# JuliaStats/Klara.jl

Hardware: AMD Instinct MI355X
Metric: MCMC transitions/sec (whole node), 100-dim Gaussian, 65k chains (higher is better)
Workload: dtype f64

## Files before the change

klara.jl_amd/csrc/klara_diagt.h:

```cpp
#pragma once
#include "klara_kernels.h"
#include "klara_mala_screen.h"

#ifndef KLARA_DIAGT_Q
#define KLARA_DIAGT_Q 8
#endif
#define KLARA_DIAGT_CPW (64 / KLARA_DIAGT_Q)
#ifndef KLARA_DT_FENCE_EVERY
#define KLARA_DT_FENCE_EVERY 2
#endif
#ifndef KLARA_DT_SLICE_WF
#define KLARA_DT_SLICE_WF 4
#endif
#ifndef KLARA_DT_W1
#define KLARA_DT_W1 4
#endif
#ifndef KLARA_Q4_MALA_WF
#define KLARA_Q4_MALA_WF 3
#endif
#ifndef KLARA_Q4_SCTAB_WF
#define KLARA_Q4_SCTAB_WF 3
#endif
#ifndef KLARA_DT_WF
#define KLARA_DT_WF 2
// ... 198 lines not shown
    constexpr int CH = KLARA_DT_RMW_CHUNK;
#pragma unroll
    for (int p0 = 0; p0 < NP; p0 += CH) {
        kd_uint4 ts[CH], tq[CH];
#pragma unroll
        for (int k = 0; k < CH; ++k) {
            if (p0 + k < NP) {
                const unsigned o = fold ? pair_off<NP, Q>(c, p0 + k) : KLARA_BUF_OOB;
                ts[k] = __builtin_amdgcn_raw_buffer_load_b128(wsum, o, 0, 0);
                tq[k] = __builtin_amdgcn_raw_buffer_load_b128(wsq, o, 0, 0);
            }
        }
#pragma unroll
        for (int k = 0; k < CH; ++k) {
            if (p0 + k < NP) {
                const int p = p0 + k;
                const unsigned o = fold ? pair_off<NP, Q>(c, p) : KLARA_BUF_OOB;
                const double s0 = __builtin_bit_cast(double, kd_uint2{ ts[k].x, ts[k].y }) + hf * x[2 * p];
                const double s1 = __builtin_bit_cast(double, kd_uint2{ ts[k].z, ts[k].w }) + hf * x[2 * p + 1];
                const double q0 = __builtin_bit_cast(double, kd_uint2{ tq[k].x, tq[k].y }) + hf * (x[2 * p] * x[2 * p]);
                const double q1 = __builtin_bit_cast(double, kd_uint2{ tq[k].z, tq[k].w }) + hf * (x[2 * p + 1] * x[2 * p + 1]);
                const kd_uint2 a = __builtin_bit_cast(kd_uint2, s0), b = __builtin_bit_cast(kd_uint2, s1);
                const kd_uint2 e = __builtin_bit_cast(kd_uint2, q0), f = __builtin_bit_cast(kd_uint2, q1);
                if (p < NP - 1) {
                    __builtin_amdgcn_raw_buffer_store_b128(kd_uint4{ a.x, a.y, b.x, b.y }, wsum, o, 0, 0);
                    __builtin_amdgcn_raw_buffer_store_b128(kd_uint4{ e.x, e.y, f.x, f.y }, wsq, o, 0, 0);
                } else {
                    const unsigned o1 = (fold && c.last_full) ? o + 8u : KLARA_BUF_OOB;
                    __builtin_amdgcn_raw_buffer_store_b64(a, wsum, o, 0, 0); __builtin_amdgcn_raw_buffer_store_b64(b, wsum, o1, 0, 0);
                    __builtin_amdgcn_raw_buffer_store_b64(e, wsq, o, 0, 0); __builtin_amdgcn_raw_buffer_store_b64(f, wsq, o1, 0, 0);
                }
            }
        }
    }
    held = fold ? 0 : held;
}

template <int NP, int Q>
__device__ __forceinline__ void load_pair_param(const PairCtx<NP, Q>& c, const gdouble* base, int D, double dflt, double (&v)[2 * NP])
{
#pragma unroll
    for (int p = 0; p < NP; ++p) {
        const int i = 2 * (p * Q + c.q);
        v[2 * p] = dflt; v[2 * p + 1] = dflt;
        if (base != nullptr && i < D) v[2 * p] = base[i];
        if (base != nullptr && i + 1 < D) v[2 * p + 1] = base[i + 1];
    }
}

template <int Q> struct PairShare {
    static constexpr int STEP = Q <= 8 ? 8 / Q : 0;
    static constexpr bool second(int p) { return STEP != 0 && ((p / (STEP ? STEP : 1)) & 1) != 0; }
};
template <int NP, int Q>
__device__ __forceinline__ void pair_words(const PairCtx<NP, Q>& c, unsigned long long seed, unsigned long long gchain,
                                           unsigned long long t, int p, uint32_t (&stash)[4], uint32_t& wa, uint32_t& wb)
{
    constexpr int STEP = PairShare<Q>::STEP, S1 = STEP ? STEP : 1;
    if (PairShare<Q>::second(p)) {
        wa = stash[2 * (p % S1)]; wb = stash[2 * (p % S1) + 1];
    } else {
        const uint32_t idx = (uint32_t)(p * Q + c.q);
        const bool pad = p == NP - 1 && !c.last_ok;
        const kd_u32x4 b = kd_stream_block(seed, gchain, t, pad ? idx : kd_pair_block(idx));
        if constexpr (STEP != 0) {
            wa = b.x; wb = b.y;
            stash[2 * (p % S1)] = b.z; stash[2 * (p % S1) + 1] = b.w;
        } else {
            const bool hb = !pad && kd_pair_half(idx) != 0u;
            wa = hb ? b.z : b.x; wb = hb ? b.w : b.y;
        }
    }
}
template <int NP, int Q, bool SCTAB = false>
__device__ __forceinline__ void pair_normals(const PairCtx<NP, Q>& c, unsigned long long seed, unsigned long long gchain,
                                             unsigned long long t, int p, uint32_t (&stash)[4], double& z0, double& z1, double& u1, double& lg1)
{
    uint32_t wa, wb;
    pair_words<NP, Q>(c, seed, gchain, t, p, stash, wa, wb);
    kd_normal_pair_w_t<SCTAB>(wa, wb, &z0, &z1, &u1, &lg1);
    KLARA_PIN(z0); KLARA_PIN(z1);
    if (p == NP - 1 && !c.last_ok) z0 = 0.0;
    if (p == NP - 1 && !c.last_full) z1 = 0.0;
}
template <int NP, int Q>
__device__ __forceinline__ void pair_issue(const PairCtx<NP, Q>& c, unsigned long long seed, unsigned long long gchain,
                                           unsigned long long t, int p, uint32_t (&stash)[4], kd_pair_reads& rd)
{
    uint32_t wa, wb;
    pair_words<NP, Q>(c, seed, gchain, t, p, stash, wa, wb);
    kd_normal_pair_issue(wa, wb, &rd);
    __builtin_amdgcn_sched_barrier(0);
}
template <int NP, int Q>
__device__ __forceinline__ void pair_issue_log(const PairCtx<NP, Q>& c, unsigned long long seed, unsigned long long gchain,
                                               unsigned long long t, int p, uint32_t (&stash)[4], kd_pair_reads& rd, uint32_t& wb)
{
    uint32_t wa;
    pair_words<NP, Q>(c, seed, gchain, t, p, stash, wa, wb);
    kd_normal_pair_issue_log(wa, wb, &rd);
    __builtin_amdgcn_sched_barrier(0);
}
__device__ __forceinline__ void pair_issue_angle(uint32_t wb, kd_pair_reads& rd)
{
    kd_normal_pair_issue_angle(wb, &rd);
    __builtin_amdgcn_sched_barrier(0);
}
template <int NP, int Q>
__device__ __forceinline__ void pair_finish(const PairCtx<NP, Q>& c, int p, const kd_pair_reads& rd, double& z0, double& z1, double& u1, double& lg1)
{
    kd_normal_pair_finish(&rd, &z0, &z1, &u1, &lg1);
    KLARA_PIN(z0); KLARA_PIN(z1);
    if (p == NP - 1 && !c.last_ok) z0 = 0.0;
    if (p == NP - 1 && !c.last_full) z1 = 0.0;
}

template <int V> struct kd_int { static constexpr int value = V; };
template <int FROM, int TO, class F>
__device__ __forceinline__ void kd_static_for(F&& f)
{
    if constexpr (FROM < TO) { f(kd_int<FROM>{}); kd_static_for<FROM + 1, TO>(f); }
}

template <bool UNITW>
__device__ __forceinline__ void diag_elem(double x, double w, double m2w, double m, double& term, double& grad)
{
    const double dd = UNITW ? x : x - m;
    term = UNITW ? dd * dd : w * (dd * dd);
    grad = UNITW ? -2.0 * dd : m2w * dd;
}

template <int SAMPLER, int NP, int Q, bool ONESTEP, bool TUNE, bool SCTAB = false>
__host__ __device__ constexpr int diagt_min_waves()
{
    return SCTAB && Q == 4 && NP > 8 ? KLARA_Q4_SCTAB_WF
         : NP <= 8 ? (ONESTEP && SAMPLER != KLARA_SAMPLER_HMC ? KLARA_DT_W1 : KLARA_DT_WF)
                   : (Q == 4 && NP <= 13 && !TUNE ? (SAMPLER == KLARA_SAMPLER_MALA ? KLARA_Q4_MALA_WF : 2) : 1);
}

#ifndef KLARA_SCTAB_MIN_STEPS
#define KLARA_SCTAB_MIN_STEPS 8
#endif
template <int SAMPLER, int NP, int Q, bool ONESTEP, bool UNITW, bool MON, bool TUNE>
__host__ __device__ constexpr bool diagt_sctab()
{
    return SAMPLER == KLARA_SAMPLER_MALA && ((Q == 4 && NP == 13) || (Q == 8 && NP == 7)) && !ONESTEP && UNITW && MON && !TUNE;
}
#ifndef KLARA_MALA_SCREEN
#define KLARA_MALA_SCREEN 1
#endif
#ifndef KLARA_MALA_SCREEN_RUN
#define KLARA_MALA_SCREEN_RUN 2
#endif
template <bool C, class A, class B> struct kd_type_if { typedef A type; };
template <class A, class B> struct kd_type_if<false, A, B> { typedef B type; };
template <int SAMPLER, int NP, int Q, bool UNITW, bool TUNE, bool USERPAIR, bool SCTAB>
__host__ __device__ constexpr bool diagt_mala_screen()
{
    return KLARA_MALA_SCREEN != 0 && SCTAB && SAMPLER == KLARA_SAMPLER_MALA && Q == 4 && NP == 13 && UNITW && !TUNE && !USERPAIR;
}
#ifndef KLARA_Q4_SCTAB_WG
#define KLARA_Q4_SCTAB_WG 256
#endif
template <int Q, bool SCTAB>
__host__ __device__ constexpr int diagt_wg_threads() { return SCTAB && Q == 4 ? KLARA_Q4_SCTAB_WG : 256; }
#ifndef KLARA_Q4_KEPT_MEANS
#define KLARA_Q4_KEPT_MEANS 0
#endif
#ifndef KLARA_Q8_KEPT_MEANS
#define KLARA_Q8_KEPT_MEANS 0
#endif
template <int SAMPLER, int NP, int Q, bool UNITW, bool TUNE, bool SCTAB>
__host__ __device__ constexpr int diagt_kept_means()
{
    return SCTAB && SAMPLER == KLARA_SAMPLER_MALA && UNITW && !TUNE ? (Q == 4 ? KLARA_Q4_KEPT_MEANS : Q == 8 ? KLARA_Q8_KEPT_MEANS : 0) : 0;
}

#ifdef KLARA_USER_PAIR_TARGET
#define KLARA_PAIR_CALL(a, b, P, g0, g1) klara_user_pair((a), (b), (P), D, (const double*)p.cdata, (long long)p.cndata, (g0), (g1))
#else
#define KLARA_PAIR_CALL(a, b, P, g0, g1) 0.0
#endif
template <int SAMPLER, int NP, int Q, bool ONESTEP, bool UNITW, bool MON, bool TUNE = false, bool DA = false, bool USERPAIR = false, bool SCTAB = false>
__global__ __launch_bounds__((diagt_wg_threads<Q, SCTAB>()), (SAMPLER == KLARA_SAMPLER_SLICE && NP <= 8 && !MON && !TUNE ? KLARA_DT_SLICE_WF : diagt_min_waves<SAMPLER, NP, Q, ONESTEP, TUNE, SCTAB>()))
void k_diagt(const KParams* __restrict__ pp, const KLaunch kl, const KAuto ka)
{
#ifndef KLARA_USER_PAIR_TARGET
    static_assert(!USERPAIR, "pair closures exist in run-time compiled translation units only");
#endif
    static_assert(!USERPAIR || (UNITW && Q >= 8), "pair closures: 8 or more lanes per chain");
    static_assert(!SCTAB || (!ONESTEP && !USERPAIR && SAMPLER != KLARA_SAMPLER_SLICE), "the remainder table: fused launches of the built-in MH / MALA / HMC kernels");
    if (ka.cell_in != nullptr && *ka.cell_in != ka.my_mode) return;
    static_assert(!(ONESTEP && (MON || TUNE)), "monitored / tuned jobs run the committing kernel");
    static_assert(!DA || (TUNE && SAMPLER == KLARA_SAMPLER_HMC), "dual averaging: tuned HMC");
    constexpr bool PLAIN = !TUNE;
    constexpr int E = 2 * NP, CPW = 64 / Q;
    constexpr bool NEEDG = SAMPLER == KLARA_SAMPLER_MALA || SAMPLER == KLARA_SAMPLER_HMC;
    constexpr bool SLICE = SAMPLER == KLARA_SAMPLER_SLICE;
    constexpr int KM = diagt_kept_means<SAMPLER, NP, Q, UNITW, TUNE, SCTAB>();
    static_assert(KM >= 0 && KM <= E, "kept drift means: a prefix of the lane's elements");
    constexpr bool SCREEN = diagt_mala_screen<SAMPLER, NP, Q, UNITW, TUNE, USERPAIR, SCTAB>();
    static_assert(!(SLICE && ONESTEP), "the slice sampler moves every chain: it runs the committing kernel");
    constexpr bool MEMSUM = MON && !TUNE && Q == 4 && (SAMPLER == KLARA_SAMPLER_MH || SAMPLER == KLARA_SAMPLER_MALA);
    const KParams& p = *pp;
    __shared__ __attribute__((aligned(16))) double lds_w[UNITW ? 2 : 2 * NP * Q];
    __shared__ __attribute__((aligned(16))) double lds_mu[UNITW ? 2 : 2 * NP * Q];
    __shared__ __attribute__((aligned(16))) double lds_m2w[UNITW ? 2 : 2 * NP * Q];
    if (!UNITW) {
        for (int i = (int)threadIdx.x; i < 2 * NP * Q; i += (int)blockDim.x) {
            lds_w[i] = (p.gw != nullptr && i < p.D) ? p.gw[i] : 1.0;
            lds_mu[i] = (p.gmu != nullptr && i < p.D) ? p.gmu[i] : 0.0;
            lds_m2w[i] = -2.0 * lds_w[i];
        }
    }
    __shared__ __attribute__((aligned(16))) double lds_screen[6];
    if constexpr (SCREEN) {
        if (threadIdx.x == 0) {
            const kd_mala_screen_k k = kd_mala_screen_consts(p.step0, p.sqrt_step0, 0.5 * p.inv_step0);
            lds_screen[0] = k.K0; lds_screen[1] = k.K1; lds_screen[4] = k.K2; lds_screen[5] = 0.0;
            lds_screen[2] = k.on ? k.T0 : __builtin_nan(""); lds_screen[3] = k.on ? k.T2 : __builtin_nan("");
        }
    }
    auto_begin();
    if constexpr (SCTAB) kd_sincos_rem_to_lds();
    kd_tables_to_lds();
    if (p.clock_probe != nullptr && blockIdx.x == (gridDim.x >> 1) && threadIdx.x == 0) {
        p.clock_probe[2] = __builtin_amdgcn_s_memtime(); p.clock_probe[3] = __builtin_amdgcn_s_memrealtime();
    }
    const int D = p.D;
    const PairCtx<NP, Q> cx = make_pctx<NP, Q>(D);
    const int nsteps = ONESTEP ? 1 : kl.nsteps;
    guchar* const accept_out = p.accept != nullptr ? p.accept + kl.t0 * (unsigned long long)p.nchains : nullptr;

    double sig[E];
    const auto wv = [&](int e) { return UNITW ? 1.0 : lds_w[2 * ((e >> 1) * Q + cx.q) + (e & 1)]; };
    const auto mv = [&](int e) { return UNITW ? 0.0 : lds_mu[2 * ((e >> 1) * Q + cx.q) + (e & 1)]; };
    const auto m2wv = [&](int e) { return UNITW ? -2.0 : lds_m2w[2 * ((e >> 1) * Q + cx.q) + (e & 1)]; };
    const auto wvl = [&](int e) { return UNITW ? 1.0 : *(volatile const double*)&lds_w[2 * ((e >> 1) * Q + cx.q) + (e & 1)]; };
    const auto mvl = [&](int e) { return UNITW ? 0.0 : *(volatile const double*)&lds_mu[2 * ((e >> 1) * Q + cx.q) + (e & 1)]; };
    const auto m2wvl = [&](int e) { return UNITW ? -2.0 : *(volatile const double*)&lds_m2w[2 * ((e >> 1) * Q + cx.q) + (e & 1)]; };
    if (SAMPLER == KLARA_SAMPLER_MH) load_pair_param<NP, Q>(cx, p.vecparam, D, 1.0, sig);
    const double gconst = USERPAIR ? 0.0 : p.gconst;

    const int acc_slot = (D + 1) >> 1;
    const bool acc_free = acc_slot < NP * Q && !PairShare<Q>::second(NP - 1);
    const int acc_lane = (cx.lane - cx.q) + (acc_slot & (Q - 1));

    const long long nwaves = (long long)gridDim.x * (blockDim.x >> 6);
    const long long wave0 = __builtin_amdgcn_readfirstlane((int)(blockIdx.x * (blockDim.x >> 6) + (threadIdx.x >> 6)));
    unsigned wave_acc = 0;
    KLARA_DT_GROUP_LOOP {
        const long long first_chain = grp * CPW;
        const long long left = p.nchains - first_chain;
        const int here = left < CPW ? (int)left : CPW;
        const bool chain_ok = cx.cw < here;
        const long long chain = first_chain + cx.cw;
        const unsigned long long gchain = (unsigned long long)(p.chain_offset + chain);
        const __amdgpu_buffer_rsrc_t wx = group_window(p.X, first_chain, here, D);
        const __amdgpu_buffer_rsrc_t wg = group_window(p.GR, first_chain, here, D);

        double x[E];
        load_pairs<NP, Q>(cx, wx, x);
        const auto late_ctx = [&]() -> PairCtx<NP, Q> {
            if constexpr (SCTAB && Q == 4) {
                int l = (int)__builtin_amdgcn_mbcnt_hi(~0u, __builtin_amdgcn_mbcnt_lo(~0u, 0u));
                KLARA_PIN(l);
                return make_pctx_at<NP, Q>(D, l & 63);
            } else return cx;
        };
        const auto user_pair = [&](int pi, double a, double b, double& nt, double& g0, double& g1) {
            double u0 = 0.0, u1 = 0.0, u = 0.0;
            const bool ok0 = pi < NP - 1 || cx.last_ok, ok1 = pi < NP - 1 || cx.last_full;
            if (ok0) u = KLARA_PAIR_CALL(a, b, pi * Q + cx.q, &u0, &u1);
            nt = ok0 ? -u : 0.0; g0 = ok0 ? u0 : 0.0; g1 = ok1 ? u1 : 0.0;
        };
        const auto grad_of = [&](const double (&v)[E], double (&out)[E]) {
            if constexpr (USERPAIR) {
#pragma unroll
                for (int pi = 0; pi < NP; ++pi) { double nt; user_pair(pi, v[2 * pi], v[2 * pi + 1], nt, out[2 * pi], out[2 * pi + 1]); }
            } else {
#pragma unroll
                for (int e = 0; e < E; ++e) { double term_; diag_elem<UNITW>(v[e], wv(e), m2wv(e), mv(e), term_, out[e]); }
            }
        };
        double lt = p.LT[chain_ok ? chain : 0];
        typename kd_type_if<SCREEN, unsigned, unsigned long long>::type nacc = 0;
        bool stuck = false;
        const bool do_sum = MON && p.sum != nullptr;
        double sm[MEMSUM ? 2 : E], sq[MEMSUM ? 2 : E];
        bool sums_loaded = false;
        long long held = 0;
        __amdgpu_buffer_rsrc_t wsum = wx, wsq = wx;
        if (do_sum) {
#pragma unroll
            for (int e = 0; e < (MEMSUM ? 2 : E); ++e) { sm[e] = 0.0; sq[e] = 0.0; }
            wsum = group_window(p.sum, first_chain, here, D); wsq = group_window(p.sumsq, first_chain, here, D);
            held = p.held[chain_ok ? chain : 0];
        }
        int sphase = kl.save_phase0;
        long long scol = kl.save_col0;
        const bool per_chain_tune = KCNT && !KPOOLED;
        const long long c0 = chain_ok ? chain : 0;
        TuneRegs tn;
        if (per_chain_tune) tn = { p.tune_step[c0], p.tune_accepted[c0], p.tune_proposed[c0], p.tune_totproposed[c0], 0, 0.0, 0.0 };
        else if (KPOOLED) tn = { p.tune_step[0], p.tune_accepted[0], 0, 0, 0, 0.0, 0.0 };
        else tn = { DA ? p.tune_step[c0] : p.step0, 0, 0, 0, 0, 0.0, 0.0 };
        if (DA) { tn.epsbar = p.da_epsbar[c0]; tn.hbar = p.da_hbar[c0]; }
        const long long acc0 = tn.accepted;
        tn.phase = per_chain_tune ? (int)(tn.proposed % p.period) : 0;

        struct { unsigned long long seed; long long hist_cols, held_inc; int thinning, acc_free, save_lo, save_hi; double sqrt_step0, half_inv_step0; } lc = {};
        if constexpr (SCTAB) {
            lc.seed = p.seed; lc.hist_cols = p.hist_cols; lc.thinning = (int)p.thinning;
            lc.held_inc = __builtin_amdgcn_readfirstlane(do_sum ? 1 : 0); lc.sqrt_step0 = p.sqrt_step0;
            KLARA_PIN_S(lc.seed); KLARA_PIN_S(lc.hist_cols); KLARA_PIN_S(lc.thinning);
            KLARA_PIN_S(lc.held_inc); KLARA_PIN_S(lc.sqrt_step0);
            const kd_uint2 hih = __builtin_bit_cast(kd_uint2, 0.5 * p.inv_step0);
            lc.half_inv_step0 = __builtin_bit_cast(double, kd_uint2{ (uint32_t)__builtin_amdgcn_readfirstlane((int)hih.x), (uint32_t)__builtin_amdgcn_readfirstlane((int)hih.y) });
            KLARA_PIN_S(lc.half_inv_step0);
            lc.acc_free = __builtin_amdgcn_readfirstlane(acc_free ? 1 : 0);
            KLARA_PIN_S(lc.acc_free);
            const long long lo = (long long)p.burnin - (long long)kl.t0, hi = (long long)p.nsteps_total - (long long)kl.t0;
            lc.save_lo = (int)(lo < 0 ? 0 : lo > nsteps ? nsteps : lo); lc.save_hi = (int)(hi < 0 ? 0 : hi > nsteps ? nsteps : hi);
            KLARA_PIN_S(lc.save_lo); KLARA_PIN_S(lc.save_hi);
        }
#define KLARA_LC(f) (SCTAB ? lc.f : p.f)
        double dm[KM > 0 ? KM : 1];
        const double neg_h_kept = KM > 0 ? -tn.step : 0.0;
        if constexpr (KM > 0) {
#pragma unroll
            for (int e = 0; e < KM; ++e) dm[e] = x[e] + neg_h_kept * x[e];
        }
        double sxx = 0.0;
        int srun = 0;
        if constexpr (SCREEN) {
#pragma unroll
            for (int e = 0; e < E; ++e) sxx = kd_fma(x[e], x[e], sxx);
        }
        for (int s = 0; s < nsteps; ++s) {
            const unsigned long long t = kl.t0 + (unsigned long long)s;
            if (KCNT) tune_count_proposal(p, tn);
            double xp[E];
            const auto put_xp = [&](int pi, double a, double b) { xp[2 * pi] = a; xp[2 * pi + 1] = b; };
            constexpr int NR = Q == 4 ? 2 : 1;
            double red[3 * NR] = {}, red1[1], red2[2];
            double u_last = 0.5, lg_last = 0.0;
            uint32_t nstash[4] = { 0u, 0u, 0u, 0u };
            bool acc;
            double ltp, a_da = 0.0;

            constexpr bool ZFIRST = (ONESTEP || Q != 4) && SAMPLER != KLARA_SAMPLER_HMC && !SLICE;
            double z[ZFIRST ? E : 2];
            kd_pair_reads rd[2];
            if (ZFIRST) {
                if constexpr (SCTAB) pair_issue<NP, Q>(cx, KLARA_LC(seed), gchain, t, 0, nstash, rd[0]);
#pragma unroll
                for (int pi = 0; pi < NP; ++pi) {
                    if constexpr (SCTAB) {
                        if (pi + 1 < NP) pair_issue<NP, Q>(cx, KLARA_LC(seed), gchain, t, pi + 1, nstash, rd[(pi + 1) & 1]);
                        pair_finish<NP, Q>(cx, pi, rd[pi & 1], z[2 * pi], z[2 * pi + 1], u_last, lg_last);
                        __builtin_amdgcn_sched_barrier(0);
                    } else {
                        pair_normals<NP, Q, SCTAB>(cx, KLARA_LC(seed), gchain, t, pi, nstash, z[2 * pi], z[2 * pi + 1], u_last, lg_last);
                        KLARA_DT_PAIR_FENCE(pi);
                    }
                }
            }
            if constexpr (SLICE) {
                if (do_sum && __any(held > 0))
                    diagt_fold<NP, Q>(cx, wsum, wsq, held > 0, sums_loaded, held, x, sm, sq);
            }
            if (SLICE) {
                acc = true;
                const __amdgpu_buffer_rsrc_t wwid = __builtin_amdgcn_make_buffer_rsrc((void*)p.vecparam, 0, D * 8, 0x00020000);
#pragma unroll
                for (int e = 0; e < E; ++e) {
                    const int i = 2 * ((e >> 1) * Q + cx.q) + (e & 1);
                    const bool live = chain_ok && i < D;
                    const uint32_t base = (uint32_t)(live ? i : 0) << KLARA_SLICE_ATT_BITS;
                    const kd_u32x4 b0 = kd_stream_block(KLARA_LC(seed), gchain, t, base);
                    const double lgu = kd_log_u01(kd_uniform_xy(b0));
                    const double ru = kd_uniform_zw(b0);
                    const double wi_t = UNITW ? 1.0 : wv(e), mi_t = UNITW ? 0.0 : mv(e);
                    const double xi = x[e], wd = __builtin_bit_cast(double, __builtin_amdgcn_raw_buffer_load_b64(wwid, (unsigned)(live ? i : 0) * 8u, 0, 0));
                    double tcur, gd_;
                    if constexpr (USERPAIR) { double g1_; user_pair(e >> 1, x[e & ~1], x[e | 1], tcur, gd_, g1_); }
                    else diag_elem<UNITW>(xi, wi_t, -2.0 * wi_t, mi_t, tcur, gd_);
                    double Li = xi - ru * wd;
                    double Ri = xi + (1.0 - ru) * wd;
                    const auto term_of = [&](double cand) -> double {
                        double tc, gd;
                        if constexpr (USERPAIR) { double g1; user_pair(e >> 1, (e & 1) ? x[e & ~1] : cand, (e & 1) ? cand : x[e | 1], tc, gd, g1); }
                        else diag_elem<UNITW>(cand, wi_t, -2.0 * wi_t, mi_t, tc, gd);
                        return tc;
                    };
                    if (p.stepout) {
                        double dl = tcur - term_of(Li);
                        int guard = 0;
                        while (true) {
                            bool go = live && !stuck && (dl > lgu);
                            if (go && ++guard > KLARA_SLICE_MAX_ATT) { stuck = true; go = false; }
                            if (!__any(go)) break;
                            const double Ln = Li - wd;
                            const double dn = tcur - term_of(go ? Ln : Li);
                            if (go) { Li = Ln; dl = dn; }
                        }
                        double dr = tcur - term_of(Ri);
                        guard = 0;
                        while (true) {
                            bool go = live && !stuck && (dr > lgu);
                            if (go && ++guard > KLARA_SLICE_MAX_ATT) { stuck = true; go = false; }
                            if (!__any(go)) break;
                            const double Rn = Ri + wd;
                            const double dn = tcur - term_of(go ? Rn : Ri);
                            if (go) { Ri = Rn; dr = dn; }
                        }
                    }
                    double xprime = xi;
                    bool done = !live || stuck;
                    kd_u32x4 ab = b0;
                    for (uint32_t a = 1;; ++a) {
                        if (!done && a > KLARA_SLICE_MAX_ATT) { stuck = true; done = true; }
                        if (!__any(!done)) break;
                        if (a & 1u) ab = kd_stream_block(KLARA_LC(seed), gchain, t, kd_slice_attempt_slot(base, a));
                        const double u = (a & 1u) ? kd_uniform_xy(ab) : kd_uniform_zw(ab);
                        const double cand = u * (Ri - Li) + Li;
                        const double tc = term_of(done ? xprime : cand);
                        if (!done) {
                            xprime = cand;
                            if (tcur - tc > lgu) done = true;
                            else if (cand > xi) Ri = cand;
                            else if (cand < xi) Li = cand;
                            else { stuck = true; done = true; }
                        }
                    }
                    if (live && !stuck) x[e] = xprime;
                }
                red1[0] = 0.0;
                if constexpr (USERPAIR) {
#pragma unroll
                    for (int pi = 0; pi < NP; ++pi) { double nt, g0_, g1_; user_pair(pi, x[2 * pi], x[2 * pi + 1], nt, g0_, g1_); red1[0] = red1[0] + nt; }
                } else {
#pragma unroll
                for (int e = 0; e < E; ++e) { double te, gd; diag_elem<UNITW>(x[e], wv(e), m2wv(e), mv(e), te, gd); red1[0] = red1[0] + te; }
                }
                group_allreduce<1>(red1, Q, cx.lane);
                lt = gconst - red1[0];
                ltp = lt;
#pragma unroll
                for (int e = 0; e < E; ++e) xp[e] = x[e];
            } else if (SAMPLER == KLARA_SAMPLER_MH) {
                const auto mh_elem = [&](int e, double ze, int r) -> double {
                    const double xe = x[e] + sig[e] * ze;
                    double term, gd;
                    diag_elem<UNITW>(xe, wv(e), m2wv(e), mv(e), term, gd);
                    red[r] = red[r] + term;
                    return xe;
                };
#pragma unroll
                for (int pi = 0; pi < NP; ++pi) {
                    double z0 = ZFIRST ? z[(2 * pi) % (ZFIRST ? E : 2)] : 0.0, z1 = ZFIRST ? z[(2 * pi + 1) % (ZFIRST ? E : 2)] : 0.0;
                    if (!ZFIRST) pair_normals<NP, Q, SCTAB>(cx, KLARA_LC(seed), gchain, t, pi, nstash, z0, z1, u_last, lg_last);
                    const int r = (NR == 2 && (pi & 1)) ? 3 : 0;
                    if constexpr (USERPAIR) {
                        const double a = x[2 * pi] + sig[2 * pi] * z0, b = x[2 * pi + 1] + sig[2 * pi + 1] * z1;
                        double nt, g0, g1;
                        user_pair(pi, a, b, nt, g0, g1);
                        red[r] = red[r] + nt;
                        put_xp(pi, a, b);
                    } else {
                        const double a = mh_elem(2 * pi, z0, r), b = mh_elem(2 * pi + 1, z1, r);
                        put_xp(pi, a, b);
                    }
                    if (!ZFIRST) KLARA_DT_PAIR_FENCE(pi);
                }
                if (NR == 2) {
                    red2[0] = red[0]; red2[1] = red[3];
                    group_allreduce<2>(red2, Q, cx.lane);
                    red1[0] = red2[0] + red2[1];
                } else {
                    red1[0] = red[0];
                    group_allreduce<1>(red1, Q, cx.lane);
                }
                ltp = gconst - red1[0];
                const double ratio = ltp - lt;
                acc = ratio > 0.0;
                if (acc_free) acc = acc || ratio > lane_bcast(lg_last, acc_lane);
                else if (!acc && ratio > KD_LOG_UMIN_GUARD)
                    acc = ratio > kd_log_u01(kd_accept_uniform(kd_stream_block(KLARA_LC(seed), gchain, t, (uint32_t)acc_slot)));
            } else if (SAMPLER == KLARA_SAMPLER_MALA) {
                const double h_ = tn.step, halfh = 0.5 * h_, sq = KCNT ? __builtin_sqrt(h_) : KLARA_LC(sqrt_step0);
                const double half_inv_h = SCTAB ? lc.half_inv_step0 : 0.5 * (KCNT ? 1.0 / h_ : p.inv_step0);
                const double neg_h = -h_;
                constexpr bool FROM_TERM = UNITW && PLAIN;
                const auto mala_elem = [&](int e, double ze, int r, bool first) -> double {
                    double term, ge = 0.0, gpe;
                    if constexpr (!UNITW) diag_elem<UNITW>(x[e], wv(e), m2wv(e), mv(e), term, ge);
                    const double m_ = UNITW ? (e < KM ? dm[e < KM ? e : 0] : x[e] + neg_h * x[e]) : x[e] + halfh * ge;
                    const double xe = m_ + sq * ze;
                    diag_elem<UNITW>(xe, wv(e), m2wv(e), mv(e), term, gpe);
                    red[r] = first ? term : red[r] + term;
                    const double q1 = m_ - xe;
                    red[r + 1] = first ? (q1 * q1) * half_inv_h : red[r + 1] + (q1 * q1) * half_inv_h;
                    const double mup = UNITW ? xe + neg_h * xe : xe + halfh * gpe;
                    const double q2 = mup - x[e];
                    red[r + 2] = first ? (q2 * q2) * half_inv_h : red[r + 2] + (q2 * q2) * half_inv_h;
                    return xe;
                };
                bool screened = false;
                if constexpr (SCREEN) {
                    double sxz = 0.0, szz = 0.0;
                    kd_screm_t sk01, skt;
                    double sk2;
                    pair_issue<NP, Q>(cx, KLARA_LC(seed), gchain, t, 0, nstash, rd[0]);
#pragma unroll
                    for (int pi = 0; pi < NP; ++pi) {
                        double z0, z1;
                        uint32_t wb_next = 0u;
                        if (pi == NP - 1) {
                            typedef volatile const __attribute__((address_space(3))) kd_screm_t* lds_entry;
                            sk01 = *(lds_entry)&lds_screen[0]; skt = *(lds_entry)&lds_screen[2];
                            sk2 = *(volatile const __attribute__((address_space(3))) double*)&lds_screen[4];
                            __builtin_amdgcn_sched_barrier(0);
                        }
                        if (pi + 1 < NP) pair_issue_log<NP, Q>(cx, KLARA_LC(seed), gchain, t, pi + 1, nstash, rd[(pi + 1) & 1], wb_next);
                        pair_finish<NP, Q>(cx, pi, rd[pi & 1], z0, z1, u_last, lg_last);
                        if (pi + 1 < NP) pair_issue_angle(wb_next, rd[(pi + 1) & 1]);
                        sxz = kd_fma(x[2 * pi], z0, sxz); sxz = kd_fma(x[2 * pi + 1], z1, sxz);
                        szz = kd_fma(z0, z0, szz); szz = kd_fma(z1, z1, szz);
                        put_xp(pi, z0, z1);
                        __builtin_amdgcn_sched_barrier(0);
                    }
                    double sc[2] = { kd_mala_screen_e(sk01.x, sk01.y, sk2, sxx, sxz, szz), kd_mala_screen_t(skt.x, skt.y, sxx, szz) };
                    group_allreduce<2>(sc, Q, cx.lane);
                    double lg_s;
                    if (lc.acc_free != 0) lg_s = lane_bcast(lg_last, acc_lane);
                    else { lg_s = KD_LOG_UMIN_GUARD; KLARA_PIN_S(lg_s); }
                    const bool certain = !chain_ok || kd_mala_screen_decide(sc[0], sc[1], lt, gconst, lg_s, nullptr, nullptr) != 0;
                    screened = __all(certain) != 0;
                    if (KLARA_MALA_SCREEN_RUN > 0 && srun >= KLARA_MALA_SCREEN_RUN) screened = false;
                    srun = screened ? srun + 1 : 0;
                    KLARA_PIN(srun);
                    acc = false; ltp = lt;
                }
                if (!screened) {
#pragma unroll
                for (int pi = 0; pi < NP; ++pi) {
                    double z0 = ZFIRST ? z[(2 * pi) % (ZFIRST ? E : 2)] : 0.0, z1 = ZFIRST ? z[(2 * pi + 1) % (ZFIRST ? E : 2)] : 0.0;
                    if constexpr (SCREEN) { z0 = xp[2 * pi]; z1 = xp[2 * pi + 1]; }
                    else if constexpr (!ZFIRST && SCTAB) {
                        if (pi == 0) pair_issue<NP, Q>(cx, KLARA_LC(seed), gchain, t, 0, nstash, rd[0]);
                        pair_finish<NP, Q>(cx, pi, rd[pi & 1], z0, z1, u_last, lg_last);
                        if (pi + 1 < NP) pair_issue<NP, Q>(cx, KLARA_LC(seed), gchain, t, pi + 1, nstash, rd[(pi + 1) & 1]);
                    } else if (!ZFIRST) pair_normals<NP, Q, SCTAB>(cx, KLARA_LC(seed), gchain, t, pi, nstash, z0, z1, u_last, lg_last);
                    const int r = (NR == 2 && (pi & 1)) ? 3 : 0;
                    if constexpr (USERPAIR) {
                        double nt, ge0, ge1, gp0, gp1;
                        user_pair(pi, x[2 * pi], x[2 * pi + 1], nt, ge0, ge1);
                        const double m0 = x[2 * pi] + halfh * ge0, m1 = x[2 * pi + 1] + halfh * ge1;
                        const double a = m0 + sq * z0, b = m1 + sq * z1;
                        user_pair(pi, a, b, nt, gp0, gp1);
                        red[r] = red[r] + nt;
                        const double q10 = m0 - a, q11 = m1 - b;
                        red[r + 1] = red[r + 1] + (q10 * q10) * half_inv_h;
                        red[r + 1] = red[r + 1] + (q11 * q11) * half_inv_h;
                        const double q20 = (a + halfh * gp0) - x[2 * pi], q21 = (b + halfh * gp1) - x[2 * pi + 1];
                        red[r + 2] = red[r + 2] + (q20 * q20) * half_inv_h;
                        red[r + 2] = red[r + 2] + (q21 * q21) * half_inv_h;
                        put_xp(pi, a, b);
                    } else {
                        const double a = mala_elem(2 * pi, z0, r, FROM_TERM && pi < NR), b = mala_elem(2 * pi + 1, z1, r, false);
                        put_xp(pi, a, b);
                    }
                    if constexpr (SCREEN) { }
                    else if constexpr (!ZFIRST && SCTAB) __builtin_amdgcn_sched_barrier(0);
                    else if (!ZFIRST) KLARA_DT_PAIR_FENCE(pi);
                }
                group_allreduce<3 * NR>(red, Q, cx.lane);
                if (NR == 2) { red[0] = red[0] + red[3]; red[1] = red[1] + red[4]; red[2] = red[2] + red[5]; }
                ltp = gconst - red[0];
                double ratio = ltp - lt;
                ratio += red[1];
                ratio -= red[2];
                acc = ratio > 0.0;
                if (SCTAB ? lc.acc_free != 0 : acc_free) acc = acc || ratio > lane_bcast(lg_last, acc_lane);
                else {
                    double guard = KD_LOG_UMIN_GUARD;
                    if constexpr (SCTAB) KLARA_PIN_S(guard);
                    if (!acc && ratio > guard)
                        acc = ratio > kd_log_u01(kd_accept_uniform(kd_stream_block(KLARA_LC(seed), gchain, t, (uint32_t)acc_slot)));
                }
                }
            } else {
                const double eps = tn.step, halfe = 0.5 * eps;
                double mom[E], gp[E];
                double k0[NR] = {};
#pragma unroll
                for (int pi = 0; pi < NP; ++pi) {
                    pair_normals<NP, Q, SCTAB>(cx, KLARA_LC(seed), gchain, t, pi, nstash, mom[2 * pi], mom[2 * pi + 1], u_last, lg_last);
                    const int r = (NR == 2 && (pi & 1)) ? 1 : 0;
                    k0[r] = k0[r] + mom[2 * pi] * mom[2 * pi];
                    k0[r] = k0[r] + mom[2 * pi + 1] * mom[2 * pi + 1];
                }
                group_allreduce<NR>(k0, Q, cx.lane);
                if (NR == 2) k0[0] = k0[0] + k0[1];
                const double H0 = lt - 0.5 * k0[0];
#pragma unroll
                for (int e = 0; e < E; ++e) xp[e] = x[e];
                constexpr bool KFOLD = UNITW && !USERPAIR;
                if constexpr (!KFOLD) grad_of(x, gp);
                const int nl = DA ? (chain_ok ? da_nleaps(p, eps) : 1) : p.nleaps;
#pragma unroll
                for (int e = 0; e < E; ++e) {
                    if constexpr (KFOLD) mom[e] = kd_fma(-eps, x[e], mom[e]);
                    else mom[e] = kd_fma(halfe, gp[e], mom[e]);
                }
                const int nlmax = DA ? wave_max_int(nl) : nl;
                for (int l = 0; l < nlmax; ++l) {
                    const bool go = !DA || l < nl;
                    const double kf = l + 1 < nl ? eps : halfe;
                    const double nkf2 = -2.0 * kf;
                    if constexpr (USERPAIR) {
#pragma unroll
                        for (int pi = 0; pi < NP; ++pi) {
                            const double xa = kd_fma(eps, mom[2 * pi], xp[2 * pi]), xb = kd_fma(eps, mom[2 * pi + 1], xp[2 * pi + 1]);
                            xp[2 * pi] = go ? xa : xp[2 * pi]; xp[2 * pi + 1] = go ? xb : xp[2 * pi + 1];
                            double nt, ga, gb;
                            user_pair(pi, xp[2 * pi], xp[2 * pi + 1], nt, ga, gb);
                            gp[2 * pi] = go ? ga : gp[2 * pi]; gp[2 * pi + 1] = go ? gb : gp[2 * pi + 1];
                            const double na = kd_fma(kf, gp[2 * pi], mom[2 * pi]), nb = kd_fma(kf, gp[2 * pi + 1], mom[2 * pi + 1]);
                            mom[2 * pi] = go ? na : mom[2 * pi]; mom[2 * pi + 1] = go ? nb : mom[2 * pi + 1];
                        }
                    } else {
#pragma unroll
                        for (int e = 0; e < E; ++e) {
                            const double x1 = kd_fma(eps, mom[e], xp[e]);
                            xp[e] = go ? x1 : xp[e];
                            if constexpr (KFOLD) {
                                const double m2 = kd_fma(nkf2, xp[e], mom[e]);
                                mom[e] = go ? m2 : mom[e];
                            } else {
                                double term, g1;
                                diag_elem<UNITW>(xp[e], 1.0, m2wvl(e), mvl(e), term, g1);
                                gp[e] = go ? g1 : gp[e];
                                const double m2 = kd_fma(kf, gp[e], mom[e]);
                                mom[e] = go ? m2 : mom[e];
                            }
                        }
                    }
                }
                if constexpr (USERPAIR) {
#pragma unroll
                    for (int pi = 0; pi < NP; ++pi) {
                        double nt, ga, gb;
                        user_pair(pi, xp[2 * pi], xp[2 * pi + 1], nt, ga, gb);
                        red[0] = red[0] + nt;
                        red[1] = red[1] + mom[2 * pi] * mom[2 * pi];
                        red[1] = red[1] + mom[2 * pi + 1] * mom[2 * pi + 1];
                    }
                } else {
#pragma unroll
                for (int e = 0; e < E; ++e) {
                    double term, gd;
                    diag_elem<UNITW>(xp[e], wv(e), m2wv(e), mv(e), term, gd);
                    const int r = (NR == 2 && ((e >> 1) & 1)) ? 3 : 0;
                    red[r] = red[r] + term;
                    red[r + 1] = red[r + 1] + mom[e] * mom[e];
                }
                }
                if (NR == 2) {
                    double red4[4] = { red[0], red[1], red[3], red[4] };
                    group_allreduce<4>(red4, Q, cx.lane);
                    red2[0] = red4[0] + red4[2]; red2[1] = red4[1] + red4[3];
                } else {
                    red2[0] = red[0]; red2[1] = red[1];
                    group_allreduce<2>(red2, Q, cx.lane);
                }
                ltp = gconst - red2[0];
                const double H1 = ltp - 0.5 * red2[1];
                const double ratio = H1 - H0;
                const double ex = kd_exp(ratio);
                const double a = 1.0 < ex ? 1.0 : ex;
                a_da = a;
                const double u = acc_free ? lane_bcast(u_last, acc_lane)
                                          : kd_accept_uniform(kd_stream_block(KLARA_LC(seed), gchain, t, (uint32_t)acc_slot));
                acc = u < a;
            }

            if constexpr (SCTAB) {
                if (accept_out != nullptr) {
                    const PairCtx<NP, Q> cxa = late_ctx();
                    if (cxa.cw < here && cxa.q == 0) accept_out[(long long)s * p.nchains + (first_chain + cxa.cw)] = acc ? 1 : 0;
                }
            } else if (accept_out != nullptr && chain_ok && cx.q == 0) accept_out[(long long)s * p.nchains + chain] = acc ? 1 : 0;
            if (KCNT && acc && !SLICE) tn.accepted += 1;
            if (DA) da_update(p, tn, (long long)t + 1, a_da);
            if (per_chain_tune && !DA) tuning_block(p, tn);
            else if (DA && per_chain_tune && tn.phase == 0 && (long long)t + 1 <= p.da_nadapt) {
                tn.totproposed += tn.proposed; tn.accepted = 0; tn.proposed = 0;
            }
            if constexpr (ONESTEP) {
                wave_acc += (acc && chain_ok && cx.q == 0) ? 1u : 0u;
                if (acc) {
                    store_pairs<NP, Q>(cx, wx, xp);
                    if (NEEDG) { double gq[E]; grad_of(xp, gq); store_pairs<NP, Q>(cx, wg, gq); }
                    if (chain_ok && cx.q == 0) { p.LT[chain] = ltp; p.naccept[chain] += 1ull; }
                }
            } else {
                nacc += acc ? 1u : 0u;
                if (!SLICE && do_sum && __any(chain_ok && acc && held > 0)) {
                    const bool fold = chain_ok && acc && held > 0;
#ifdef KLARA_DT_FOLD_RMW
                    if constexpr (MEMSUM) diagt_fold_rmw<NP, Q>(cx, wsum, wsq, fold, held, x);
#else
                    if constexpr (MEMSUM) diagt_fold_atomic<NP, Q>(cx, p.sum + first_chain * D, p.sumsq + first_chain * D, fold, held, x);
#endif
                    else diagt_fold<NP, Q>(cx, wsum, wsq, fold, sums_loaded, held, x, sm, sq);
                }
                if (acc) {
#pragma unroll
                    for (int e = 0; e < E; ++e) x[e] = xp[e];
                    if constexpr (KM > 0) {
#pragma unroll
                        for (int e = 0; e < KM; ++e) dm[e] = xp[e] + neg_h_kept * xp[e];
                    }
                    if constexpr (SCREEN) {
                        sxx = 0.0;
#pragma unroll
                        for (int e = 0; e < E; ++e) sxx = kd_fma(xp[e], xp[e], sxx);
                    }
                    lt = ltp;
                }
            }
            const long long i1 = (long long)t + 1;
            if (MON && (SCTAB ? s >= lc.save_lo && s < lc.save_hi : i1 > p.burnin && i1 <= p.nsteps_total)) {
                if (sphase == 0) {
                    if constexpr (SCTAB) held += lc.held_inc;
                    else if (do_sum) held += 1;
                    if (scol < KLARA_LC(hist_cols)) {
                        const long long col0 = scol * p.nchains + first_chain;
                        const PairCtx<NP, Q> cxh = late_ctx();
                        if (p.hist != nullptr) store_pairs<NP, Q>(cxh, group_window(p.hist, col0, here, D), x);
                        if (NEEDG && p.hist_g != nullptr) { double gq[E]; grad_of(x, gq); store_pairs<NP, Q>(cxh, group_window(p.hist_g, col0, here, D), gq); }
                        if constexpr (SCTAB) {
                            if (p.hist_lt != nullptr && cxh.cw < here && cxh.q == 0) p.hist_lt[scol * p.nchains + (first_chain + cxh.cw)] = lt;
                        } else if (p.hist_lt != nullptr && chain_ok && cx.q == 0) p.hist_lt[scol * p.nchains + chain] = lt;
                    }
                    ++scol;
                }
                sphase = (sphase + 1 == (SCTAB ? lc.thinning : (int)p.thinning)) ? 0 : sphase + 1;
            }
        }
        const PairCtx<NP, Q> cxe = late_ctx();
        const bool chain_ok_e = SCTAB ? cxe.cw < here : chain_ok;
        const long long chain_e = SCTAB ? first_chain + cxe.cw : chain;
        if (do_sum) {
            if constexpr (!MEMSUM) {
                if (__any(sums_loaded)) {
                    store_pairs_if<NP, Q>(cxe, wsum, sums_loaded, sm);
                    store_pairs_if<NP, Q>(cxe, wsq, sums_loaded, sq);
                }
            }
            if (chain_ok_e && cxe.q == 0) p.held[chain_e] = held;
        }
        if (SLICE && stuck && chain_ok) klara_raise(p.error_flag, KLARA_ERR_SLICE_STUCK);
        if (!ONESTEP) wave_acc += (chain_ok_e && cxe.q == 0) ? (unsigned)nacc : 0u;
        if (!ONESTEP && nacc != 0) {
            store_pairs<NP, Q>(cxe, wx, x);
            if (NEEDG) { double gq[E]; grad_of(x, gq); store_pairs<NP, Q>(cxe, wg, gq); }
            if (chain_ok_e && cxe.q == 0) { p.LT[chain_e] = lt; p.naccept[chain_e] += nacc; }
        }
        if (TUNE && chain_ok && cx.q == 0) {
            if (DA) { p.tune_step[chain] = tn.step; p.da_epsbar[chain] = tn.epsbar; p.da_hbar[chain] = tn.hbar; }
            if (per_chain_tune) {
                p.tune_step[chain] = tn.step; p.tune_accepted[chain] = tn.accepted;
                p.tune_proposed[chain] = tn.proposed; p.tune_totproposed[chain] = tn.totproposed;
            } else if (KPOOLED && KCNT) {
                atomicAdd((unsigned long long*)p.pooled_accepted, (unsigned long long)(tn.accepted - acc0));
            }
        }
    }
    if (p.clock_probe != nullptr && blockIdx.x == (gridDim.x >> 1) && threadIdx.x == 0) {
        p.clock_probe[0] = __builtin_amdgcn_s_memtime(); p.clock_probe[1] = __builtin_amdgcn_s_memrealtime();
    }
    auto_finish(ka, wave_acc);
#undef KLARA_LC
}

template <int NP, int Q, bool USERPAIR = false>
__global__ __launch_bounds__(256) void k_diagt_init(const KParams p, int needgrad)
{
#ifndef KLARA_USER_PAIR_TARGET
    static_assert(!USERPAIR, "pair closures exist in run-time compiled translation units only");
#endif
    constexpr int E = 2 * NP, CPW = 64 / Q;
    const int D = p.D;
    const PairCtx<NP, Q> cx = make_pctx<NP, Q>(D);
    const long long grp = __builtin_amdgcn_readfirstlane((int)(blockIdx.x * (blockDim.x >> 6) + (threadIdx.x >> 6)));
    const long long first_chain = grp * CPW;
    const long long left = p.nchains - first_chain;
    const int here = left < CPW ? (left > 0 ? (int)left : 0) : CPW;
    const bool chain_ok = cx.cw < here;
    const long long chain = first_chain + cx.cw;
    double w[E], mu[E], x[E], g[E], red[1] = { 0.0 };
    load_pair_param<NP, Q>(cx, p.gw, D, 1.0, w);
    load_pair_param<NP, Q>(cx, p.gmu, D, 0.0, mu);
    load_pairs<NP, Q>(cx, group_window(p.X, first_chain, here, D), x);
    bool bad = false;
    if constexpr (USERPAIR) {
#pragma unroll
        for (int pi = 0; pi < NP; ++pi) {
            double u0 = 0.0, u1 = 0.0, u = 0.0;
            const bool ok0 = pi < NP - 1 || cx.last_ok, ok1 = pi < NP - 1 || cx.last_full;
            if (ok0) u = KLARA_PAIR_CALL(x[2 * pi], x[2 * pi + 1], pi * Q + cx.q, &u0, &u1);
            red[0] = red[0] + (ok0 ? -u : 0.0);
            g[2 * pi] = ok0 ? u0 : 0.0; g[2 * pi + 1] = ok1 ? u1 : 0.0;
            bad = bad || !kfinite(g[2 * pi]) || !kfinite(g[2 * pi + 1]);
        }
    } else {
#pragma unroll
    for (int e = 0; e < E; ++e) {
        double term;
        diag_elem<false>(x[e], w[e], -2.0 * w[e], mu[e], term, g[e]);
        red[0] = red[0] + term;
        bad = bad || !kfinite(g[e]);
    }
    }
    group_allreduce<1>(red, Q, cx.lane);
    const double lt = (USERPAIR ? 0.0 : p.gconst) - red[0];
    bad = chain_ok && ((needgrad && bad) || !kfinite(lt));
    if (needgrad) store_pairs<NP, Q>(cx, group_window(p.GR, first_chain, here, D), g);
    if (chain_ok && cx.q == 0) p.LT[chain] = lt;
    if (bad) klara_raise(p.error_flag, KLARA_ERR_NONFINITE_INIT);
}
```

klara.jl_amd/csrc/klara_mala_screen.h:

```cpp
#ifndef KLARA_MALA_SCREEN_H
#define KLARA_MALA_SCREEN_H

#include "detmath.h"

#define KD_MALA_SCREEN_H_MIN 0.015625
#define KD_MALA_SCREEN_H_MAX 2.0
#define KD_MALA_SCREEN_MARGIN 9.313225746154785e-10
#define KD_MALA_SCREEN_T_MAX 1.0715086071862673e+301
#define KD_MALA_SCREEN_ELEM_FACTOR 96.0

typedef struct {
    double K0, K1, K2;
    double T0, T2;
    int on;
} kd_mala_screen_k;

KD_FN double kd_mala_screen_abs(double v) { return __builtin_fabs(v); }

KD_FN kd_mala_screen_k kd_mala_screen_consts(double h, double s, double c)
{
    kd_mala_screen_k k;
    const double a = 1.0 - h, a2 = a * a, b = a2 - 1.0, aa = kd_mala_screen_abs(a), ab = kd_mala_screen_abs(b);
    const double cb = c * b, one_cb = 1.0 + cb, s2 = s * s;
    k.K0 = -(a2 + cb * b);
    k.K1 = -2.0 * (a * s) * one_cb;
    k.K2 = -s2 * one_cb;
    const double cross = c * ab * aa * s;
    k.T0 = a2 + aa * s + c * (b * b) + cross;
    k.T2 = s2 + aa * s + c * s2 + cross + c * (a2 * s2);
    const double mu = h + aa;
    const double exz = s * (16.0 * mu + 8.0 * aa + c * mu * (8.0 + 6.0 * mu * aa));
    const double E0 = 11.0 * (mu * mu) + 4.0 * ab + 0.5 * exz;
    const double E2 = 5.0 * s2 + 4.0 + 2.0 * a2 + 3.0 * mu * aa + 0.5 * exz;
    const double tiny = 8.881784197001252e-16;
    int on = h >= KD_MALA_SCREEN_H_MIN && h <= KD_MALA_SCREEN_H_MAX;
    on = on && kd_mala_screen_abs(s2 - h) <= tiny * h && kd_mala_screen_abs(c * h - 0.5) <= tiny;
    on = on && k.T0 >= 0.25 && k.T2 >= 0.25;
    on = on && E0 <= KD_MALA_SCREEN_ELEM_FACTOR * k.T0 && E2 <= KD_MALA_SCREEN_ELEM_FACTOR * k.T2;
    k.on = on;
    return k;
}

KD_FN double kd_mala_screen_e(double K0, double K1, double K2, double sxx, double sxz, double szz) { return kd_fma(K0, sxx, kd_fma(K1, sxz, K2 * szz)); }
KD_FN double kd_mala_screen_t(double T0, double T2, double sxx, double szz) { return kd_fma(T0, sxx, T2 * szz); }

KD_FN int kd_mala_screen_decide(double e, double ts, double lt, double gconst, double lg, double* est_out, double* t_out)
{
    const double est = (gconst - lt) + e;
    const double T = ((kd_mala_screen_abs(gconst) + kd_mala_screen_abs(lt)) + kd_mala_screen_abs(lg)) + ts;
    if (est_out) *est_out = est;
    if (t_out) *t_out = T;
    return (T <= KD_MALA_SCREEN_T_MAX) && (est + KD_MALA_SCREEN_MARGIN * T <= lg);
}

KD_FN int kd_mala_screen_certain(const kd_mala_screen_k* k, double sxx, double sxz, double szz, double lt, double gconst, double lg,
                                 double* est_out, double* t_out)
{
    const int r = kd_mala_screen_decide(kd_mala_screen_e(k->K0, k->K1, k->K2, sxx, sxz, szz), kd_mala_screen_t(k->T0, k->T2, sxx, szz),
                                        lt, gconst, lg, est_out, t_out);
    return k->on && r;
}

#endif
```

Before: 6.876 billion.

## Extend MALA acceptance screen to Q8 layout and add certain-accept shortcut

Extends the cheap MALA accept/reject screen to the Q=8, NP=7 fused kernel. It also adds a three-way decision: certain reject, certain accept, or uncertain. When every chain in a wave is certain, it takes a short proposal path that computes only the proposal's squared norm instead of the full drift and gradient work. This aims to skip the expensive Metropolis-adjusted evaluation for decisive steps, at the cost of extra reductions, branch divergence and more register pressure.

```diff
diff --git a/klara.jl_amd/csrc/klara_diagt.h b/klara.jl_amd/csrc/klara_diagt.h
--- a/klara.jl_amd/csrc/klara_diagt.h
+++ b/klara.jl_amd/csrc/klara_diagt.h
@@ -374,6 +374,20 @@
 #ifndef KLARA_MALA_SCREEN_RUN
 #define KLARA_MALA_SCREEN_RUN 2
 #endif
+#ifndef KLARA_MALA_SCREEN_ACCEPT
+#define KLARA_MALA_SCREEN_ACCEPT 1
+#endif
+#ifndef KLARA_MALA_SCREEN_Q8
+#define KLARA_MALA_SCREEN_Q8 1
+#endif
+#ifndef KLARA_MALA_SCREEN_ACCEPT_Q4
+#define KLARA_MALA_SCREEN_ACCEPT_Q4 0
+#endif
+template <int SAMPLER, int NP, int Q, bool UNITW, bool TUNE, bool USERPAIR, bool SCTAB>
+__host__ __device__ constexpr bool diagt_mala_screen8()
+{
+    return KLARA_MALA_SCREEN != 0 && KLARA_MALA_SCREEN_Q8 != 0 && SCTAB && SAMPLER == KLARA_SAMPLER_MALA && Q == 8 && NP == 7 && UNITW && !TUNE && !USERPAIR;
+}
 template <bool C, class A, class B> struct kd_type_if { typedef A type; };
 template <class A, class B> struct kd_type_if<false, A, B> { typedef B type; };
 template <int SAMPLER, int NP, int Q, bool UNITW, bool TUNE, bool USERPAIR, bool SCTAB>
@@ -422,6 +436,8 @@
     constexpr int KM = diagt_kept_means<SAMPLER, NP, Q, UNITW, TUNE, SCTAB>();
     static_assert(KM >= 0 && KM <= E, "kept drift means: a prefix of the lane's elements");
     constexpr bool SCREEN = diagt_mala_screen<SAMPLER, NP, Q, UNITW, TUNE, USERPAIR, SCTAB>();
+    constexpr bool SCREEN8 = diagt_mala_screen8<SAMPLER, NP, Q, UNITW, TUNE, USERPAIR, SCTAB>();
+    constexpr bool SCRACC = KLARA_MALA_SCREEN_ACCEPT != 0 && (Q == 8 || KLARA_MALA_SCREEN_ACCEPT_Q4 != 0);
     static_assert(!(SLICE && ONESTEP), "the slice sampler moves every chain: it runs the committing kernel");
     constexpr bool MEMSUM = MON && !TUNE && Q == 4 && (SAMPLER == KLARA_SAMPLER_MH || SAMPLER == KLARA_SAMPLER_MALA);
     const KParams& p = *pp;
@@ -436,7 +452,7 @@
         }
     }
     __shared__ __attribute__((aligned(16))) double lds_screen[6];
-    if constexpr (SCREEN) {
+    if constexpr (SCREEN || SCREEN8) {
         if (threadIdx.x == 0) {
             const kd_mala_screen_k k = kd_mala_screen_consts(p.step0, p.sqrt_step0, 0.5 * p.inv_step0);
             lds_screen[0] = k.K0; lds_screen[1] = k.K1; lds_screen[4] = k.K2; lds_screen[5] = 0.0;
@@ -555,7 +571,7 @@
         }
         double sxx = 0.0;
         int srun = 0;
-        if constexpr (SCREEN) {
+        if constexpr (SCREEN || SCREEN8) {
 #pragma unroll
             for (int e = 0; e < E; ++e) sxx = kd_fma(x[e], x[e], sxx);
         }
@@ -729,6 +745,30 @@
                     red[r + 2] = first ? (q2 * q2) * half_inv_h : red[r + 2] + (q2 * q2) * half_inv_h;
                     return xe;
                 };
+                const auto mala_elem_short = [&](int e, double ze, int r, bool first) -> double {
+                    const double m_ = e < KM ? dm[e < KM ? e : 0] : x[e] + neg_h * x[e];
+                    const double xe = m_ + sq * ze;
+                    const double term = xe * xe;
+                    red[r] = first ? term : red[r] + term;
+                    return xe;
+                };
+                bool shortp = false, sacc = false;
+                const auto screen_vote = [&](double (&sc)[2]) -> bool {
+                    group_allreduce<2>(sc, Q, cx.lane);
+                    double lg_s;
+                    if (lc.acc_free != 0) lg_s = lane_bcast(lg_last, acc_lane);
+                    else { lg_s = KD_LOG_UMIN_GUARD; KLARA_PIN_S(lg_s); }
+                    if constexpr (SCRACC) {
+                        const int dec = chain_ok ? kd_mala_screen_decide2(sc[0], sc[1], lt, gconst, lg_s, lc.acc_free, nullptr, nullptr) : KD_MALA_SCREEN_REJECTED;
+                        const bool allrej = __all(dec == KD_MALA_SCREEN_REJECTED) != 0;
+                        shortp = !allrej && __all(dec != 0) != 0;
+                        sacc = dec == KD_MALA_SCREEN_ACCEPTED;
+                        return allrej;
+                    } else {
+                        const bool certain = !chain_ok || kd_mala_screen_decide(sc[0], sc[1], lt, gconst, lg_s, nullptr, nullptr) != 0;
+                        return __all(certain) != 0;
+                    }
+                };
                 bool screened = false;
                 if constexpr (SCREEN) {
                     double sxz = 0.0, szz = 0.0;
@@ -754,16 +794,52 @@
                         __builtin_amdgcn_sched_barrier(0);
                     }
                     double sc[2] = { kd_mala_screen_e(sk01.x, sk01.y, sk2, sxx, sxz, szz), kd_mala_screen_t(skt.x, skt.y, sxx, szz) };
-                    group_allreduce<2>(sc, Q, cx.lane);
-                    double lg_s;
-                    if (lc.acc_free != 0) lg_s = lane_bcast(lg_last, acc_lane);
-                    else { lg_s = KD_LOG_UMIN_GUARD; KLARA_PIN_S(lg_s); }
-                    const bool certain = !chain_ok || kd_mala_screen_decide(sc[0], sc[1], lt, gconst, lg_s, nullptr, nullptr) != 0;
-                    screened = __all(certain) != 0;
+                    if constexpr (SCRACC) screened = screen_vote(sc);
+                    else {
+                        group_allreduce<2>(sc, Q, cx.lane);
+                        double lg_s;
+                        if (lc.acc_free != 0) lg_s = lane_bcast(lg_last, acc_lane);
+                        else { lg_s = KD_LOG_UMIN_GUARD; KLARA_PIN_S(lg_s); }
+                        const bool certain = !chain_ok || kd_mala_screen_decide(sc[0], sc[1], lt, gconst, lg_s, nullptr, nullptr) != 0;
+                        screened = __all(certain) != 0;
+                    }
                     if (KLARA_MALA_SCREEN_RUN > 0 && srun >= KLARA_MALA_SCREEN_RUN) screened = false;
                     srun = screened ? srun + 1 : 0;
                     KLARA_PIN(srun);
                     acc = false; ltp = lt;
+                }
+                if constexpr (SCREEN8) {
+                    typedef volatile const __attribute__((address_space(3))) kd_screm_t* lds_entry;
+                    const kd_screm_t sk01 = *(lds_entry)&lds_screen[0], skt = *(lds_entry)&lds_screen[2];
+                    const double sk2 = *(volatile const __attribute__((address_space(3))) double*)&lds_screen[4];
+                    double sxz = 0.0, szz = 0.0;
+#pragma unroll
+                    for (int e = 0; e < E; ++e) { sxz = kd_fma(x[e], z[e % (ZFIRST ? E : 2)], sxz); szz = kd_fma(z[e % (ZFIRST ? E : 2)], z[e % (ZFIRST ? E : 2)], szz); }
+                    double sc[2] = { kd_mala_screen_e(sk01.x, sk01.y, sk2, sxx, sxz, szz), kd_mala_screen_t(skt.x, skt.y, sxx, szz) };
+                    screened = screen_vote(sc);
+                    acc = false; ltp = lt;
+                }
+                if constexpr ((SCREEN || SCREEN8) && SCRACC) {
+                    if (shortp) {
+#pragma unroll
+                        for (int pi = 0; pi < NP; ++pi) {
+                            const double z0 = SCREEN ? xp[2 * pi] : z[(2 * pi) % (ZFIRST ? E : 2)], z1 = SCREEN ? xp[2 * pi + 1] : z[(2 * pi + 1) % (ZFIRST ? E : 2)];
+                            const int r = (NR == 2 && (pi & 1)) ? 3 : 0;
+                            const double a = mala_elem_short(2 * pi, z0, r, FROM_TERM && pi < NR), b = mala_elem_short(2 * pi + 1, z1, r, false);
+                            put_xp(pi, a, b);
+                        }
+                        if (NR == 2) {
+                            red2[0] = red[0]; red2[1] = red[3];
+                            group_allreduce<2>(red2, Q, cx.lane);
+                            red1[0] = red2[0] + red2[1];
+                        } else {
+                            red1[0] = red[0];
+                            group_allreduce<1>(red1, Q, cx.lane);
+                        }
+                        ltp = gconst - red1[0];
+                        acc = sacc;
+                        screened = true;
+                    }
                 }
                 if (!screened) {
 #pragma unroll
@@ -946,7 +1022,7 @@
 #pragma unroll
                         for (int e = 0; e < KM; ++e) dm[e] = xp[e] + neg_h_kept * xp[e];
                     }
-                    if constexpr (SCREEN) {
+                    if constexpr (SCREEN || SCREEN8) {
                         sxx = 0.0;
 #pragma unroll
                         for (int e = 0; e < E; ++e) sxx = kd_fma(xp[e], xp[e], sxx);
diff --git a/klara.jl_amd/csrc/klara_mala_screen.h b/klara.jl_amd/csrc/klara_mala_screen.h
--- a/klara.jl_amd/csrc/klara_mala_screen.h
+++ b/klara.jl_amd/csrc/klara_mala_screen.h
@@ -53,6 +53,29 @@
     return (T <= KD_MALA_SCREEN_T_MAX) && (est + KD_MALA_SCREEN_MARGIN * T <= lg);
 }
 
+#define KD_MALA_SCREEN_REJECTED 1
+#define KD_MALA_SCREEN_ACCEPTED 2
+KD_FN int kd_mala_screen_decide2(double e, double ts, double lt, double gconst, double lg, int have_draw, double* est_out, double* t_out)
+{
+    const double est = (gconst - lt) + e;
+    const double T = ((kd_mala_screen_abs(gconst) + kd_mala_screen_abs(lt)) + kd_mala_screen_abs(lg)) + ts;
+    if (est_out) *est_out = est;
+    if (t_out) *t_out = T;
+    const double mt = KD_MALA_SCREEN_MARGIN * T, la = have_draw ? lg : 0.0;
+    const int ok = T <= KD_MALA_SCREEN_T_MAX;
+    if (ok && (est + mt <= lg)) return KD_MALA_SCREEN_REJECTED;
+    if (ok && (est - mt > la)) return KD_MALA_SCREEN_ACCEPTED;
+    return 0;
+}
+
+KD_FN int kd_mala_screen_certain2(const kd_mala_screen_k* k, double sxx, double sxz, double szz, double lt, double gconst, double lg, int have_draw,
+                                  double* est_out, double* t_out)
+{
+    const int r = kd_mala_screen_decide2(kd_mala_screen_e(k->K0, k->K1, k->K2, sxx, sxz, szz), kd_mala_screen_t(k->T0, k->T2, sxx, szz),
+                                         lt, gconst, lg, have_draw, est_out, t_out);
+    return k->on ? r : 0;
+}
+
 KD_FN int kd_mala_screen_certain(const kd_mala_screen_k* k, double sxx, double sxz, double szz, double lt, double gconst, double lg,
                                  double* est_out, double* t_out)
 {
```

Result: no change. 6.902 billion, median of 2 (+0.4%).
